# pySTEPS/pysteps

Measured on AMD Instinct MI355X. Metric: Mpixels*leadsteps/s (LK+semilag) at 4096x4096 fp32, higher is better.
Workload: dtype f32

## Files before the change

### pysteps_amd/csrc/lk.hip

```cpp
#include <algorithm>
#include <cmath>
#include <cstring>
#include <functional>
#include <vector>

#include "common.h"

#pragma clang fp contract(off)

namespace psh {
namespace {

enum Stat : int {
  kMinAll = 0,
  kNanCount,
  kMaxAll,
  kMinFeat,
  kMaxFeat,
  kEigMax,
  kNumStats = 8
};

constexpr int kRedBlocks = 1024;

// ... 484 lines not shown
  __syncthreads();
  if (threadIdx.x == 0) {
    for (int w = 1; w < nwaves; ++w) {
      if (what == 0) {
        a = fmin(a, sm[0][w]);
        b += sm[1][w];
      } else {
        a = fmax(a, sm[0][w]);
        b = fmin(b, sm[1][w]);
        c = fmax(c, sm[2][w]);
      }
    }
    if (what == 0) {
      dstats[0] = a;
      stats[kMinAll] = static_cast<float>(a);
      stats[kNanCount] = static_cast<float>(b);
    } else {
      dstats[1] = a;
      dstats[2] = b;
      dstats[3] = c;
      stats[kMaxAll] = static_cast<float>(a);
      stats[kMinFeat] = static_cast<float>(b);
      stats[kMaxFeat] = static_cast<float>(c);
    }
  }
}

__global__ __launch_bounds__(256) void lk_open_bits_f64(const double *__restrict__ img, int m, int n,
                                                        int size_opening, int buffer_mask,
                                                        const float *__restrict__ stats,
                                                        const double *__restrict__ dstats,
                                                        float *__restrict__ clean32, double *__restrict__ clean64,
                                                        double *__restrict__ partial) {
  __shared__ double red[3][4];
  const double mn = dstats[0];
  const int lane = threadIdx.x & 63, wave = threadIdx.x >> 6;
  const int x = blockIdx.x * kOpenColsW - 2 + lane;
  const int yb = blockIdx.y * kOpenRowsWG + wave * kOpenRowsW;
  const bool col_in = x >= 0 && x < n;
  constexpr int kLoad = kOpenRowsW + 4;
  double v[kLoad];
#pragma unroll
  for (int q = 0; q < kLoad; ++q) {
    const int y = yb - 2 + q;
    v[q] = (col_in && y >= 0 && y < m) ? img[static_cast<size_t>(y) * n + x] : 0.0;
  }
  unsigned long long A[kLoad], F[kLoad];
#pragma unroll
  for (int q = 0; q < kLoad; ++q) {
    const int y = yb - 2 + q;
    const bool row_in = y >= 0 && y < m;
    F[q] = __ballot(row_in && col_in && isfinite(v[q]) && v[q] > mn);
    A[q] = F[q] | __ballot(!(row_in && col_in));
  }
  unsigned long long E[kLoad];
#pragma unroll
  for (int q = 1; q < kLoad - 1; ++q) E[q] = F[q] & (A[q] << 1) & (A[q] >> 1) & A[q - 1] & A[q + 1];
  double mx_all = -INFINITY, mn_feat = INFINITY, mx_feat = -INFINITY;
  const int first_row = buffer_mask > 0 ? (stats[kNanCount] > 0.f ? 2 : 1) : 0;
  const bool writer = lane >= 2 && lane < 2 + kOpenColsW && col_in;
#pragma unroll
  for (int q = 2; q < kLoad - 2; ++q) {
    const int y = yb - 2 + q;
    if (y >= m) break;
    const unsigned long long O = E[q] | (E[q] << 1) | (E[q] >> 1) | E[q - 1] | E[q + 1];
    double val = v[q];
    if (size_opening > 0 && ((F[q] >> lane) & 1ull) && !((O >> lane) & 1ull)) val = mn;
    if (writer) {
      if (isfinite(val)) {
        mx_all = fmax(mx_all, val);
        if (y >= first_row) {
          mn_feat = fmin(mn_feat, val);
          mx_feat = fmax(mx_feat, val);
        }
      }
      clean64[static_cast<size_t>(y) * n + x] = val;
      clean32[static_cast<size_t>(y) * n + x] = static_cast<float>(val);
    }
  }
  mx_all = wave_max_d(mx_all);
  mn_feat = wave_min_d(mn_feat);
  mx_feat = wave_max_d(mx_feat);
  if (lane == 0) {
    red[0][wave] = mx_all;
    red[1][wave] = mn_feat;
    red[2][wave] = mx_feat;
  }
  __syncthreads();
  if (threadIdx.x == 0) {
    const int b = blockIdx.y * gridDim.x + blockIdx.x, nb = gridDim.x * gridDim.y;
    partial[b] = fmax(fmax(red[0][0], red[0][1]), fmax(red[0][2], red[0][3]));
    partial[nb + b] = fmin(fmin(red[1][0], red[1][1]), fmin(red[1][2], red[1][3]));
    partial[2 * nb + b] = fmax(fmax(red[2][0], red[2][1]), fmax(red[2][2], red[2][3]));
  }
}

__device__ __forceinline__ unsigned char quantise_f64(double v, double lo, double hi) {
  const double s = (hi - lo) > 1e-8 ? (v - lo) / (hi - lo) * 255.0 : v - lo;
  return static_cast<unsigned char>(static_cast<int>(s));
}

__global__ __launch_bounds__(256) void lk_to_u8_f64(const double *__restrict__ clean, int m, int n, int buffer_mask,
                                                    const float *__restrict__ stats,
                                                    const double *__restrict__ dstats,
                                                    unsigned char *__restrict__ trk, unsigned char *__restrict__ feat) {
  const double fill = dstats[0], hi = dstats[1], flo = dstats[2], fhi = dstats[3];
  const int first_row = buffer_mask > 0 ? (stats[kNanCount] > 0.f ? 2 : 1) : 0;
  const size_t npx = static_cast<size_t>(m) * n;
  const size_t first_feature_px = static_cast<size_t>(first_row) * n;
  const size_t stride = static_cast<size_t>(gridDim.x) * blockDim.x;
  for (size_t p = static_cast<size_t>(blockIdx.x) * blockDim.x + threadIdx.x; p < npx; p += stride) {
    double v = clean[p];
    const bool ok = isfinite(v);
    if (!ok) v = fill;
    trk[p] = quantise_f64(v, fill, hi);
    if (feat) feat[p] = quantise_f64((ok && p >= first_feature_px) ? v : fill, flo, fhi);
  }
}

constexpr int kMaxBlockR = 3;

__device__ __forceinline__ bool px_allowed(const float *__restrict__ clean, int m, int n, int x,
                                           int y, int bm, bool any_nan) {
  if (!any_nan) return true;
  if (bm <= 0) return isfinite(clean[static_cast<size_t>(y) * n + x]);
  const int a = bm / 2;
  for (int j = 0; j < bm; ++j) {
    const int yy = y + j - a;
    if (yy < 0 || yy >= m) continue;
    for (int i = 0; i < bm; ++i) {
      const int xx = x + i - a;
      if (xx < 0 || xx >= n) continue;
      if (!isfinite(clean[static_cast<size_t>(yy) * n + xx])) return false;
    }
  }
  return true;
}

__device__ __forceinline__ float next_lane_f(float v) {
  return __int_as_float(__builtin_amdgcn_update_dpp(0, __float_as_int(v), 0x130 , 0xf, 0xf, true));
}
__device__ __forceinline__ double next_lane_d(double v) {
  const int lo = __builtin_amdgcn_update_dpp(0, __double2loint(v), 0x130, 0xf, 0xf, true);
  const int hi = __builtin_amdgcn_update_dpp(0, __double2hiint(v), 0x130, 0xf, 0xf, true);
  return __hiloint2double(hi, lo);
}
__device__ __forceinline__ bool walk_mirrored(int i, int n) {
  if (i >= 0 && i + 1 < n) return false;
  return reflect101(i + 1, n) != reflect101(reflect101(i, n) + 1, n);
}

constexpr int crn_cols(int block_size) { return 64 - 2 * (block_size / 2 + 1); }

template <int BS, int ROWS>
__global__ __launch_bounds__(256) void lk_corner_response_cols(
    const unsigned char *__restrict__ u8, const float *__restrict__ clean, int m, int n,
    int buffer_mask, const float *__restrict__ stats, float *__restrict__ eig,
    float *__restrict__ partial, Band band, unsigned *__restrict__ slots, int *__restrict__ zero_a, int count_a,
    int *__restrict__ zero_b, int count_b) {
  constexpr int r = BS / 2, H = r + 1, W = crn_cols(BS);
  if (blockIdx.x == 0 && blockIdx.y == 0) {
    for (int i = threadIdx.x; i < count_a; i += 256) zero_a[i] = 0;
    for (int i = threadIdx.x; i < count_b; i += 256) zero_b[i] = 0;
  }
  __shared__ float red[4];
  const int lane = threadIdx.x & 63, wave = __builtin_amdgcn_readfirstlane(threadIdx.x >> 6);
  const int x0 = blockIdx.x * W;
  const int yb = (blockIdx.y * 4 + wave) * ROWS;
  float best = 0.f;
  if (yb < m) {
    const float s = 1.0f / (4.0f * static_cast<float>(BS) * 255.0f), s2 = 2.f * s;
    const int xl = x0 - H + lane;
    const bool neg_x = walk_mirrored(xl + 1, n);
    const float sx = neg_x ? -s : s, sx2 = neg_x ? -s2 : s2;
    const unsigned char *col = u8 + reflect101(xl, n);
    const bool few_rows = m < 2 * H + 2;
    auto row_of = [&](int y) -> int {
      if (few_rows) return reflect101(y, m);
      y = y < 0 ? -y : y;
      return y >= m ? 2 * m - 2 - y : y;
    };
    auto load_row = [&](int i) -> int { return col[static_cast<size_t>(row_of(yb - H + i)) * n]; };
    auto row_terms = [&](int raw, float &hd, float &g) {
      const float a = static_cast<float>(raw);
      const float c = next_lane_f(a);
      const float b = next_lane_f(c);
      hd = b - a;
      g = (a + b) * s + c * s2;
    };
    const bool any_nan = stats[kNanCount] > 0.f;
    const int x = x0 + lane;
    const bool writer = lane < W && x < n;
    const int rows_out = min(ROWS, m - yb);
    const int last_p = rows_out + BS - 1;
    double ring[3][BS], V[3] = {0.0, 0.0, 0.0};
#pragma unroll
    for (int j = 0; j < BS; ++j) ring[0][j] = ring[1][j] = ring[2][j] = 0.0;
    int raw[BS];
    const int raw0 = load_row(0), raw1 = load_row(1);
#pragma unroll
    for (int j = 0; j < BS; ++j) raw[j] = load_row(2 + j);
    float hd_m, hd_0, g_m, g_0;
    row_terms(raw0, hd_m, g_m);
    row_terms(raw1, hd_0, g_0);
    for (int base = 1; base <= last_p; base += BS) {
      int nxt[BS];
#pragma unroll
      for (int j = 0; j < BS; ++j) nxt[j] = load_row(base + BS + 1 + j);
#pragma unroll
      for (int j = 0; j < BS; ++j) {
        const int p = base + j;
        if (p > last_p) break;
        constexpr int kRingBase = 1;
        const int slot = (kRingBase + j) % BS;
        float hd_p, g_p;
        row_terms(raw[j], hd_p, g_p);
        const float dx = (hd_m + hd_p) * sx + hd_0 * sx2;
        float dy = g_p - g_m;
        const int y_seq = yb - H + p;
        const bool row_mirrored = few_rows ? walk_mirrored(y_seq, m) : (y_seq < 0 || y_seq >= m);
        const unsigned row_sign = row_mirrored ? 0x80000000u : 0u;
        dy = __uint_as_float(__float_as_uint(dy) ^ row_sign);
        const double pxx = static_cast<double>(dx * dx), pxy = static_cast<double>(dx * dy);
        const double pyy = static_cast<double>(dy * dy);
        V[0] += pxx - ring[0][slot];
        V[1] += pxy - ring[1][slot];
        V[2] += pyy - ring[2][slot];
        ring[0][slot] = pxx;
        ring[1][slot] = pxy;
        ring[2][slot] = pyy;
        hd_m = hd_0;
        hd_0 = hd_p;
        g_m = g_0;
        g_0 = g_p;
        if (p >= BS) {
          double w0 = V[0], w1 = V[1], w2 = V[2];
          double t0 = V[0], t1 = V[1], t2 = V[2];
#pragma unroll
          for (int c = 0; c < 2 * r; ++c) {
            t0 = next_lane_d(t0);
            t1 = next_lane_d(t1);
            t2 = next_lane_d(t2);
            w0 += t0;
            w1 += t1;
            w2 += t2;
          }
          const int y = yb + p - BS;
          if (writer) {
            const float a = static_cast<float>(w0) * 0.5f, b = static_cast<float>(w1);
            const float c = static_cast<float>(w2) * 0.5f;
            const float e = (a + c) - sqrtf((a - c) * (a - c) + b * b);
            eig[static_cast<size_t>(y) * n + x] = e;
            if (y >= band.lo && y < band.hi && px_allowed(clean, m, n, x, y, buffer_mask, any_nan))
              best = fmaxf(best, fmaxf(e, 0.f));
          }
        }
      }
#pragma unroll
      for (int j = 0; j < BS; ++j) raw[j] = nxt[j];
    }
  }
  best = wave_max(best);
  if (lane == 0) red[wave] = best;
  __syncthreads();
  if (threadIdx.x == 0) {
    const int b = blockIdx.y * gridDim.x + blockIdx.x;
    const float b_max = fmaxf(fmaxf(red[0], red[1]), fmaxf(red[2], red[3]));
    if (slots) {
      slot_max(slots, kSlEig, b, b_max);
    } else {
      partial[b] = b_max;
    }
  }
}

constexpr int kNmsKeys = 64;

using CornerKeyT = unsigned long long;
__device__ __forceinline__ CornerKeyT nms_key(float val, unsigned addr) {
  return (static_cast<CornerKeyT>(__float_as_uint(val)) << 32) | addr;
}
__device__ __forceinline__ float prev_lane_f(float v) {
  return __int_as_float(__builtin_amdgcn_update_dpp(0, __float_as_int(v), 0x138 , 0xf, 0xf, true));
}

template <int BS, int ROWS>
__global__ __launch_bounds__(256) void lk_corner_response_nms(
    const unsigned char *__restrict__ u8, const float *__restrict__ clean, int m, int n, int buffer_mask,
    const float *__restrict__ stats, float quality, CornerKeyT *__restrict__ out, int cap, Band band,
    unsigned *__restrict__ slots, int *__restrict__ zero_b, int count_b) {
  constexpr int r = BS / 2, H = r + 1, W = crn_cols(BS);
  if (blockIdx.x == 0 && blockIdx.y == 0)
    for (int i = threadIdx.x; i < count_b; i += 256) zero_b[i] = 0;
  __shared__ float red[4];
  const int lane = threadIdx.x & 63, wave = __builtin_amdgcn_readfirstlane(threadIdx.x >> 6);
  int *over_count = reinterpret_cast<int *>(slots + kSlCand * kSlots);
  const int fixed_total = static_cast<int>(gridDim.x * gridDim.y) * 4 * kNmsKeys;
  const int my_slots = (static_cast<int>(blockIdx.y * gridDim.x + blockIdx.x) * 4 + wave) * kNmsKeys;
  const int x0 = blockIdx.x * (W - 2) - 1;
  const int yj = (blockIdx.y * 4 + wave) * ROWS;
  const int yb = yj - 1;
  float best = 0.f;
  float known = fmaxf(slots_max(slots, kSlEig), 0.f);
  int held = 0;
  if (yj < m) {
    const float s = 1.0f / (4.0f * static_cast<float>(BS) * 255.0f), s2 = 2.f * s;
    const int xl = x0 - H + lane;
    const bool neg_x = walk_mirrored(xl + 1, n);
    const float sx = neg_x ? -s : s, sx2 = neg_x ? -s2 : s2;
    const unsigned char *col = u8 + reflect101(xl, n);
    const bool few_rows = m < 2 * H + 4;
    auto row_of = [&](int y) -> int {
      if (few_rows) return reflect101(y, m);
      y = y < 0 ? -y : y;
      return y >= m ? 2 * m - 2 - y : y;
    };
    auto load_row = [&](int i) -> int { return col[static_cast<size_t>(row_of(yb - H + i)) * n]; };
    auto row_terms = [&](int raw, float &hd, float &g) {
      const float a = static_cast<float>(raw);
      const float c = next_lane_f(a);
      const float b = next_lane_f(c);
      hd = b - a;
      g = (a + b) * s + c * s2;
    };
    const bool any_nan = stats[kNanCount] > 0.f;
    const int x = x0 + lane;
    const bool in_image_col = lane < W && x >= 0 && x < n;
    const bool judged_col = lane >= 1 && lane < W - 1 && x >= 1 && x < n - 1;
    const int rows_e = min(ROWS + 2, m - yb);
    const int last_p = rows_e + BS - 1;
    double ring[3][BS], V[3] = {0.0, 0.0, 0.0};
#pragma unroll
    for (int j = 0; j < BS; ++j) ring[0][j] = ring[1][j] = ring[2][j] = 0.0;
    int raw[BS];
    const int raw0 = load_row(0), raw1 = load_row(1);
#pragma unroll
    for (int j = 0; j < BS; ++j) raw[j] = load_row(2 + j);
    float hd_m, hd_0, g_m, g_0;
    row_terms(raw0, hd_m, g_m);
    row_terms(raw1, hd_0, g_0);
    float c1 = 0.f, h1 = 0.f, t1 = 0.f, t2 = 0.f;
    for (int base = 1; base <= last_p; base += BS) {
      int nxt[BS];
#pragma unroll
      for (int j = 0; j < BS; ++j) nxt[j] = load_row(base + BS + 1 + j);
#pragma unroll
      for (int j = 0; j < BS; ++j) {
        const int p = base + j;
        if (p > last_p) break;
        constexpr int kRingBase = 1;
        const int slot = (kRingBase + j) % BS;
        float hd_p, g_p;
        row_terms(raw[j], hd_p, g_p);
        const float dx = (hd_m + hd_p) * sx + hd_0 * sx2;
        float dy = g_p - g_m;
        const int y_seq = yb - H + p;
        const bool row_mirrored = few_rows ? walk_mirrored(y_seq, m) : (y_seq < 0 || y_seq >= m);
        const unsigned row_sign = row_mirrored ? 0x80000000u : 0u;
        dy = __uint_as_float(__float_as_uint(dy) ^ row_sign);
        const double pxx = static_cast<double>(dx * dx), pxy = static_cast<double>(dx * dy);
        const double pyy = static_cast<double>(dy * dy);
        V[0] += pxx - ring[0][slot];
        V[1] += pxy - ring[1][slot];
        V[2] += pyy - ring[2][slot];
        ring[0][slot] = pxx;
        ring[1][slot] = pxy;
        ring[2][slot] = pyy;
        hd_m = hd_0;
        hd_0 = hd_p;
        g_m = g_0;
        g_0 = g_p;
        if (p >= BS) {
          double w0 = V[0], w1 = V[1], w2 = V[2];
          double q0 = V[0], q1 = V[1], q2 = V[2];
#pragma unroll
          for (int c = 0; c < 2 * r; ++c) {
            q0 = next_lane_d(q0);
            q1 = next_lane_d(q1);
            q2 = next_lane_d(q2);
            w0 += q0;
            w1 += q1;
            w2 += q2;
          }
          const int y = yb + p - BS;
          const float a = static_cast<float>(w0) * 0.5f, b = static_cast<float>(w1);
          const float c = static_cast<float>(w2) * 0.5f;
          const float e = (a + c) - sqrtf((a - c) * (a - c) + b * b);
          if (in_image_col && y >= 0 && y >= band.lo && y < band.hi && px_allowed(clean, m, n, x, y, buffer_mask, any_nan))
            best = fmaxf(best, fmaxf(e, 0.f));
          if ((p & 7) == 0) known = fmaxf(known, wave_max(best));
          const float h0 = fmaxf(prev_lane_f(e), next_lane_f(e)), t0 = fmaxf(e, h0);
          const int yr = y - 1;
          if (p >= BS + 2 && yr >= yj) {
            bool keep = judged_col && yr >= 1 && yr < m - 1 && yr >= band.lo && yr < band.hi;
            keep = keep && c1 > 0.f && c1 > known * quality;
            keep = keep && !(fmaxf(h1, fmaxf(t2, t0)) > c1);
            keep = keep && px_allowed(clean, m, n, x, yr, buffer_mask, any_nan);
            const unsigned long long mask = __ballot(keep);
            if (mask != 0ull) {
              const int cnt = __popcll(mask);
              int at = held + __popcll(mask & ((1ull << lane) - 1ull));
              if (held + cnt > kNmsKeys) {
                int base = 0;
                const int spill = held + cnt - max(held, kNmsKeys);
                if (lane == 0) base = atomicAdd(over_count, spill);
                base = __shfl(base, 0);
                if (at >= kNmsKeys) at = fixed_total + base + (at - max(held, kNmsKeys)) - my_slots;
              }
              if (keep && my_slots + at < cap) out[my_slots + at] = nms_key(c1, static_cast<unsigned>(yr + band.y_org) * n + x);
              held += cnt;
            }
          }
// ... 560 lines not shown
      for (int r = 0; r < ROWS; ++r) {
        if (r < row_count) {
          const int i00 = from_next_lane(ti[r + 1]), i01 = from_next_lane(i00);
          const int i10 = from_next_lane(ti[r + 2]), i11 = from_next_lane(i10);
          const int g00 = tg[r], g01 = from_next_lane(tg[r]), g10 = tg[r + 1], g11 = from_next_lane(tg[r + 1]);
          if (sample_lane) {
            const int ival = descale(bilin24(i00, i01, i10, i11, w00, w01, w10, w11), 14 - 5);
            const int gx = descale(bilin24(static_cast<short>(g00), static_cast<short>(g01), static_cast<short>(g10),
                                           static_cast<short>(g11), w00, w01, w10, w11), 14);
            const int gy = descale(bilin24(g00 >> 16, g01 >> 16, g10 >> 16, g11 >> 16, w00, w01, w10, w11), 14);
            rI[r] = static_cast<short>(ival);
            rGx[r] = static_cast<short>(gx);
            rGy[r] = static_cast<short>(gy);
            s11 += gx * gx;
            s12 += gx * gy;
            s22 += gy * gy;
          }
        }
      }
    }
    const long long a11 = wave_sum_split_i64(s11), a12 = wave_sum_split_i64(s12), a22 = wave_sum_split_i64(s22);
    if (lane == 0) {
      red[0][wave] = a11;
      red[1][wave] = a12;
      red[2][wave] = a22;
    }
    __syncthreads();
    const float flt_scale = 1.f / 1048576.f;
    const float A11 = static_cast<float>(red[0][0] + red[0][1] + red[0][2] + red[0][3]) * flt_scale;
    const float A12 = static_cast<float>(red[1][0] + red[1][1] + red[1][2] + red[1][3]) * flt_scale;
    const float A22 = static_cast<float>(red[2][0] + red[2][1] + red[2][2] + red[2][3]) * flt_scale;
    float D = A11 * A22 - A12 * A12;
    const float min_eig = (A22 + A11 - sqrtf((A11 - A22) * (A11 - A22) + 4.f * A12 * A12)) /
                          static_cast<float>(2 * win_w * win_h);
    if (min_eig < min_eig_thr || D < 1.1920929e-07f) {
      if (level == 0) ok = false;
      continue;
    }
    D = 1.f / D;
    float qx = nx - half_x, qy = ny - half_y;
    float prev_dx = 0.f, prev_dy = 0.f;
    for (int j = 0; j < max_count; ++j) {
      const int inx = static_cast<int>(floorf(qx)), iny = static_cast<int>(floorf(qy));
      if (iny < L.vlo || iny + win_h + 1 > L.vhi) suspect = true;
      if (inx < -win_w || inx >= L.cols || iny < -win_h || iny >= L.rows) {
        if (level == 0) ok = false;
        break;
      }
      lk_weights(qx - static_cast<float>(inx), qy - static_cast<float>(iny), w00, w01, w10, w11);
      const int y0 = iny + row_first;
      const bool inside = row_count > 0 && inx >= 0 && inx + 63 < L.cols && y0 >= 0 && y0 + ROWS < L.rows &&
                          y0 >= L.row_org && y0 + ROWS - L.row_org < L.rows_stored;
      int tj[ROWS + 1];
      if (inside) {
        const unsigned char *base = L.J + static_cast<size_t>(y0 - L.row_org) * L.cols + (inx + lane);
#pragma unroll
        for (int r = 0; r <= ROWS; ++r) tj[r] = base[static_cast<size_t>(r) * L.cols];
      } else {
        const int xa = reflect101(inx + lane, L.cols);
#pragma unroll
        for (int r = 0; r <= ROWS; ++r)
          tj[r] = L.J[stored_row(L, reflect101(y0 + min(r, max(row_count, 0)), L.rows)) * L.cols + xa];
      }
      int c1 = 0, c2 = 0;
      int right = from_next_lane(tj[0]);
#pragma unroll
      for (int r = 0; r < ROWS; ++r) {
        const int right_below = from_next_lane(tj[r + 1]);
        const int diff = descale(bilin24(tj[r], right, tj[r + 1], right_below, w00, w01, w10, w11), 14 - 5) - rI[r];
        c1 += __mul24(diff, rGx[r]);
        c2 += __mul24(diff, rGy[r]);
        right = right_below;
      }
      const long long b1 = wave_sum_split_i64(c1), b2 = wave_sum_split_i64(c2);
      long long (*rb)[4] = red_b[j & 1];
      if (lane == 0) {
        rb[0][wave] = b1;
        rb[1][wave] = b2;
      }
      __syncthreads();
      const float B1 = static_cast<float>(rb[0][0] + rb[0][1] + rb[0][2] + rb[0][3]) * flt_scale;
      const float B2 = static_cast<float>(rb[1][0] + rb[1][1] + rb[1][2] + rb[1][3]) * flt_scale;
      const float dx = (A12 * B2 - A22 * B1) * D;
      const float dy = (A12 * B1 - A11 * B2) * D;
      qx += dx;
      qy += dy;
      nx = qx + half_x;
      ny = qy + half_y;
      if (dx * dx + dy * dy <= eps2) break;
      if (j > 0 && fabsf(dx + prev_dx) < 0.01f && fabsf(dy + prev_dy) < 0.01f) {
        nx -= dx * 0.5f;
        ny -= dy * 0.5f;
        break;
      }
      prev_dx = dx;
      prev_dy = dy;
    }
    if (level == 0 && ok) {
      const int rx = static_cast<int>(rintf(nx - half_x)), ry = static_cast<int>(rintf(ny - half_y));
      if (ry < L.vlo || ry + win_h + 1 > L.vhi) suspect = true;
      if (rx < -win_w || rx >= L.cols || ry < -win_h || ry >= L.rows) ok = false;
    }
  }
  if (tid == 0) {
    next_pts[p] = make_float2(nx, ny);
    status[p] = (ok ? 1 : 0) | (suspect ? 2 : 0);
  }
}

__global__ __launch_bounds__(256) void lk_pool_append(const float2 *__restrict__ pts,
                                                      const float2 *__restrict__ next_pts,
                                                      const unsigned char *__restrict__ status, int npts,
                                                      const int *__restrict__ npts_dev,
                                                      double2 *__restrict__ pool_xy,
                                                      double2 *__restrict__ pool_uv,
                                                      int *__restrict__ pool_count, int capacity) {
  __shared__ int wave_total[4];
  __shared__ int running;
  const int tid = threadIdx.x, lane = tid & 63, wave = tid >> 6;
  if (npts_dev) npts = min(npts, *npts_dev);
  if (tid == 0) running = *pool_count;
  __syncthreads();
  for (int i0 = 0; i0 < npts; i0 += 256) {
    const int i = i0 + tid;
    const bool keep = i < npts && status[i] != 0;
    const unsigned long long mask = __ballot(keep);
    if (lane == 0) wave_total[wave] = __popcll(mask);
    __syncthreads();
    int pos = running;
    for (int w = 0; w < wave; ++w) pos += wave_total[w];
    pos += __popcll(mask & ((1ull << lane) - 1ull));
    if (keep && pos < capacity) {
      const float2 p = pts[i], q = next_pts[i];
      pool_xy[pos] = make_double2(p.x, p.y);
      pool_uv[pos] = make_double2(static_cast<double>(q.x - p.x), static_cast<double>(q.y - p.y));
    }
    __syncthreads();
    if (tid == 0) running += wave_total[0] + wave_total[1] + wave_total[2] + wave_total[3];
    __syncthreads();
  }
  if (tid == 0) *pool_count = running;
}

}

dim3 lk_open_grid(int m, int n) { return dim3((n + kOpenColsW - 1) / kOpenColsW, (m + kOpenRowsWG32 - 1) / kOpenRowsWG32); }
void launch_lk_open(dim3 grid, hipStream_t stream, const float *img, int m, int n, int size_opening, int buffer_mask,
                    float *stats, float *clean, float *part, Band band, unsigned *slots = nullptr,
                    unsigned long long *keepbits = nullptr) {
  hipLaunchKernelGGL(lk_open_bits, grid, dim3(256), 0, stream, img, m, n, size_opening, buffer_mask, stats, clean, part,
                     band, slots, keepbits);
}

constexpr int kCrnRows = 32;
dim3 lk_response_grid(int m, int n, int block_size) {
  const int w = crn_cols(block_size), rows = 4 * kCrnRows;
  return dim3((n + w - 1) / w, (m + rows - 1) / rows);
}
dim3 lk_response_nms_grid(int m, int n, int block_size) {
  const int w = crn_cols(block_size) - 2, rows = 4 * kCrnRows;
  return dim3((n + w - 1) / w, (m + rows - 1) / rows);
}
int lk_response_nms_fixed_keys(dim3 grid) { return static_cast<int>(grid.x * grid.y) * 4 * kNmsKeys; }
void launch_lk_response_nms(dim3 grid, hipStream_t stream, int block_size, const unsigned char *u8, const float *clean, int m,
                            int n, int buffer_mask, const float *stats, float quality, CornerKeyT *out, int cap, Band band,
                            unsigned *slots, int *zero_b, int count_b) {
#define PSH_NMS_LAUNCH(BS)                                                                                             \
  hipLaunchKernelGGL((lk_corner_response_nms<BS, kCrnRows>), grid, dim3(256), 0, stream, u8, clean, m, n, buffer_mask, \
                     stats, quality, out, cap, band, slots, zero_b, count_b)
  if (block_size == 1) {
    PSH_NMS_LAUNCH(1);
  } else if (block_size == 3) {
    PSH_NMS_LAUNCH(3);
  } else if (block_size == 5) {
    PSH_NMS_LAUNCH(5);
  } else {
    PSH_NMS_LAUNCH(7);
  }
#undef PSH_NMS_LAUNCH
}
void launch_lk_response(dim3 grid, hipStream_t stream, int block_size, const unsigned char *u8, const float *clean, int m,
                        int n, int buffer_mask, const float *stats, float *eig, float *part, Band band,
                        unsigned *slots = nullptr, int *zero_a = nullptr, int count_a = 0, int *zero_b = nullptr,
                        int count_b = 0) {
#define PSH_CRN_LAUNCH(BS)                                                                                          \
  hipLaunchKernelGGL((lk_corner_response_cols<BS, kCrnRows>), grid, dim3(256), 0, stream, u8, clean, m, n, buffer_mask, \
                     stats, eig, part, band, slots, zero_a, count_a, zero_b, count_b)
  if (block_size == 1) {
    PSH_CRN_LAUNCH(1);
  } else if (block_size == 3) {
    PSH_CRN_LAUNCH(3);
  } else if (block_size == 5) {
    PSH_CRN_LAUNCH(5);
  } else {
    PSH_CRN_LAUNCH(7);
  }
#undef PSH_CRN_LAUNCH
}

static int ensure_lk_ws(size_t nbytes, void **ptr) {
  static void *ws = nullptr;
  const int rc = persistent_device(&ws, nbytes);
  *ptr = ws;
  return rc;
}

size_t lk_prepare_ws_bytes(int m, int n, bool f64) {
  const size_t npx = static_cast<size_t>(m) * n;
  if (f64) {
    const dim3 ogrid((n + kOpenColsW - 1) / kOpenColsW, (m + kOpenRowsWG - 1) / kOpenRowsWG);
    return (npx + 2 * static_cast<size_t>(kRedBlocks) + 3 * static_cast<size_t>(ogrid.x * ogrid.y) + 8) * sizeof(double);
  }
  const dim3 ogrid = lk_open_grid(m, n);
  return kSlotBytes + sizeof(float) * (2 * static_cast<size_t>(kRedBlocks) + 3 * static_cast<size_t>(ogrid.x * ogrid.y));
}
size_t lk_slot_bytes() { return kSlotBytes; }
size_t lk_keepbits_bytes(int m, int n) { return static_cast<size_t>(m) * lk_open_grid(m, n).x * sizeof(unsigned long long); }

int lk_prepare_on(hipStream_t stream, void *ws, const void *frame_dev, bool f64, int m, int n, int size_opening,
                  int buffer_mask, float *clean_dev, unsigned char *track_u8_dev, unsigned char *feature_u8_dev,
                  float *stats_dev, unsigned *slots_cleared, unsigned long long *keepbits) {
  if (m <= 0 || n <= 0) return fail(PSH_EINVAL, "lk_prepare: invalid shape (%d,%d)", m, n);
  if (!frame_dev || !track_u8_dev || !stats_dev || !ws) return fail(PSH_EINVAL, "lk_prepare: NULL pointer");
  if (!clean_dev && (f64 || !keepbits)) return fail(PSH_EINVAL, "lk_prepare: NULL pointer");
  if (size_opening != 0 && size_opening != 3)
    return fail(PSH_EUNSUPPORTED, "lk_prepare: size_opening %d not implemented (0 or 3)", size_opening);
  const size_t npx = static_cast<size_t>(m) * n;
  if (!f64) {
    const float *frame = static_cast<const float *>(frame_dev);
    const dim3 ogrid = lk_open_grid(m, n);
    unsigned *own_slots = static_cast<unsigned *>(ws);
    float *part1 = reinterpret_cast<float *>(static_cast<char *>(ws) + kSlotBytes);
    float *part2 = part1 + 2 * kRedBlocks;
    unsigned *slots = slots_cleared;
    if (!slots) {
      slots = own_slots;
      const hipError_t e = hipMemsetAsync(slots, 0, kSlotBytes, stream);
      if (e != hipSuccess) return fail(PSH_EHIP, "lk_prepare: clearing the statistic slots failed: %s", hipGetErrorString(e));
    }
    hipLaunchKernelGGL(lk_stats1, dim3(kRedBlocks), dim3(256), 0, stream, frame, npx, part1, slots);
    if (clean_dev) {
      launch_lk_open(ogrid, stream, frame, m, n, size_opening, buffer_mask, stats_dev, clean_dev, part2, Band{0, 0, m}, slots);
      const int qgrid = static_cast<int>(std::min<size_t>((npx / 4 + 255) / 256 + 1, 4096));
      hipLaunchKernelGGL(lk_to_u8, dim3(qgrid), dim3(256), 0, stream, clean_dev, m, n, buffer_mask, stats_dev, track_u8_dev,
                         feature_u8_dev, 0, static_cast<const unsigned *>(slots));
    } else {
      launch_lk_open(ogrid, stream, frame, m, n, size_opening, buffer_mask, stats_dev, nullptr, part2, Band{0, 0, m}, slots,
                     keepbits);
      const dim3 qgrid((n + 1023) / 1024, (m + kU8Rows - 1) / kU8Rows);
      const bool vec = n % 4 == 0 && reinterpret_cast<uintptr_t>(frame) % 16 == 0 &&
                       reinterpret_cast<uintptr_t>(track_u8_dev) % 4 == 0 && reinterpret_cast<uintptr_t>(feature_u8_dev) % 4 == 0;
      if (vec) {
        hipLaunchKernelGGL(lk_to_u8_bits<true>, qgrid, dim3(256), 0, stream, frame, keepbits, static_cast<int>(ogrid.x), m, n,
                           buffer_mask, stats_dev, track_u8_dev, feature_u8_dev, static_cast<const unsigned *>(slots));
      } else {
        hipLaunchKernelGGL(lk_to_u8_bits<false>, qgrid, dim3(256), 0, stream, frame, keepbits, static_cast<int>(ogrid.x), m, n,
                           buffer_mask, stats_dev, track_u8_dev, feature_u8_dev, static_cast<const unsigned *>(slots));
      }
    }
  } else {
    const double *frame = static_cast<const double *>(frame_dev);
    const dim3 ogrid((n + kOpenColsW - 1) / kOpenColsW, (m + kOpenRowsWG - 1) / kOpenRowsWG);
    const int nb_open = ogrid.x * ogrid.y;
    double *clean64 = static_cast<double *>(ws);
    double *part1 = clean64 + npx, *part2 = part1 + 2 * kRedBlocks, *dstats = part2 + 3 * nb_open;
    hipLaunchKernelGGL(lk_stats1_f64, dim3(kRedBlocks), dim3(256), 0, stream, frame, npx, part1);
    hipLaunchKernelGGL(lk_final_f64, dim3(1), dim3(kFinalThreads), 0, stream, part1, kRedBlocks, 0, stats_dev, dstats);
    hipLaunchKernelGGL(lk_open_bits_f64, ogrid, dim3(256), 0, stream, frame, m, n, size_opening, buffer_mask, stats_dev,
                       dstats, clean_dev, clean64, part2);
    hipLaunchKernelGGL(lk_final_f64, dim3(1), dim3(kFinalThreads), 0, stream, part2, nb_open, 1, stats_dev, dstats);
    const int qgrid = static_cast<int>(std::min<size_t>((npx + 255) / 256, 8192));
    hipLaunchKernelGGL(lk_to_u8_f64, dim3(qgrid), dim3(256), 0, stream, clean64, m, n, buffer_mask, stats_dev, dstats,
                       track_u8_dev, feature_u8_dev);
  }
  const hipError_t e = hipGetLastError();
  if (e != hipSuccess) return fail(PSH_EHIP, "lk_prepare launch failed: %s", hipGetErrorString(e));
  return PSH_OK;
}


}

using psh::ctx;
using psh::fail;

extern "C" {

int psh_lk_prepare_dev(const float *frame_dev, int m, int n, int size_opening, int buffer_mask,
                       float *clean_dev, unsigned char *track_u8_dev,
                       unsigned char *feature_u8_dev, float *stats_dev) {
  PSH_REQUIRE_INIT();
  psh::Context &c = ctx();
  std::lock_guard<std::recursive_mutex> lock(c.mu);
  PSH_HIP(hipSetDevice(c.device));
  if (m <= 0 || n <= 0) return fail(PSH_EINVAL, "lk_prepare: invalid shape (%d,%d)", m, n);
  void *ws = nullptr;
  if (int rc = psh::ensure_lk_ws(psh::lk_prepare_ws_bytes(m, n, false), &ws)) return rc;
  return psh::lk_prepare_on(c.stream, ws, frame_dev, false, m, n, size_opening, buffer_mask, clean_dev, track_u8_dev,
                            feature_u8_dev, stats_dev);
}

int psh_lk_prepare_f64_dev(const double *frame_dev, int m, int n, int size_opening, int buffer_mask,
                           float *clean_dev, unsigned char *track_u8_dev,
                           unsigned char *feature_u8_dev, float *stats_dev) {
  PSH_REQUIRE_INIT();
  psh::Context &c = ctx();
  std::lock_guard<std::recursive_mutex> lock(c.mu);
  PSH_HIP(hipSetDevice(c.device));
  if (m <= 0 || n <= 0) return fail(PSH_EINVAL, "lk_prepare: invalid shape (%d,%d)", m, n);
  void *blk = nullptr;
  if (int rc = psh_malloc(&blk, psh::lk_prepare_ws_bytes(m, n, true))) return rc;
  const int rc = psh::lk_prepare_on(c.stream, blk, frame_dev, true, m, n, size_opening, buffer_mask, clean_dev,
                                    track_u8_dev, feature_u8_dev, stats_dev);
  (void)psh_free(blk);
  return rc;
}

static int check_band(const char *who, int m, int n, int e0, int e1, int r0, int r1) {
  if (m <= 0 || n <= 0 || e0 < 0 || e1 > m || e0 >= e1 || r0 < e0 || r1 > e1 || r0 > r1)
    return fail(PSH_EINVAL, "%s: rows [%d,%d) / band [%d,%d) do not fit a %d-row frame", who, r0, r1, e0, e1, m);
  return PSH_OK;
}

int psh_lk_band_stats_dev(const float *frame_dev, int m, int n, int r0, int r1, float *stats_dev) {
  PSH_REQUIRE_INIT();
  if (!frame_dev || !stats_dev) return fail(PSH_EINVAL, "lk_band_stats: NULL pointer");
  if (int rc = check_band("lk_band_stats", m, n, r0, r1, r0, r1)) return rc;
  psh::Context &c = ctx();
  std::lock_guard<std::recursive_mutex> lock(c.mu);
  PSH_HIP(hipSetDevice(c.device));
  void *ws = nullptr;
  if (int rc = psh::ensure_lk_ws(sizeof(float) * 2 * psh::kRedBlocks, &ws)) return rc;
  float *part = static_cast<float *>(ws);
  hipLaunchKernelGGL(psh::lk_stats1, dim3(psh::kRedBlocks), dim3(256), 0, c.stream,
                     frame_dev + static_cast<size_t>(r0) * n, static_cast<size_t>(r1 - r0) * n, part,
                     static_cast<unsigned *>(nullptr));
  hipLaunchKernelGGL(psh::lk_stats1_final, dim3(1), dim3(psh::kFinalThreads), 0, c.stream, part, psh::kRedBlocks, stats_dev);
  PSH_HIP(hipGetLastError());
  return PSH_OK;
// ... 796 lines not shown
```

Baseline: 282,100.

## Process two columns per lane in corner response kernel with packed loads

Restructures the corner-response kernel so each lane handles C=2 adjacent columns, with packed 16-bit byte loads on interior tiles and vectorized float2 stores. The horizontal box sum becomes a sliding window across lane-shifted values. The ring buffer now stores fp32 products instead of doubles to cut register pressure, and rows per wave go from 32 to 36. The goals are fewer DPP shuffles and memory transactions per pixel and less halo waste, at the cost of more registers per lane and more complex boundary handling.

```diff
diff --git a/pysteps_amd/csrc/lk.hip b/pysteps_amd/csrc/lk.hip
--- a/pysteps_amd/csrc/lk.hip
+++ b/pysteps_amd/csrc/lk.hip
@@ -660,112 +660,208 @@
 
 constexpr int crn_cols(int block_size) { return 64 - 2 * (block_size / 2 + 1); }
 
-template <int BS, int ROWS>
+constexpr int crn_geom_e(int r, int c) { return ((c - 1 - r) % c + c) % c; }
+template <int BS, int C>
+struct CrnGeom {
+  static constexpr int r = BS / 2;
+  static constexpr int E = crn_geom_e(r, C);
+  static constexpr int lead = 1 + E + r;
+  static constexpr int NT = C + 2 * r;
+  static constexpr int px_lanes = (E + C + 1) / C;
+  static constexpr int look = (NT - 1) / C + px_lanes;
+  static constexpr int lanes = 64 - look;
+  static constexpr int cols = C * lanes;
+  static_assert(lead % C == 0, "loads and stores of a lane are aligned together");
+};
+constexpr int kCrnC = 2;
+constexpr int kCrnRows = 36;
+constexpr int crn_strip_cols(int block_size) {
+  const int r = block_size / 2, e = crn_geom_e(r, kCrnC);
+  return kCrnC * (64 - ((kCrnC + 2 * r - 1) / kCrnC + (e + kCrnC + 1) / kCrnC));
+}
+
+__device__ __forceinline__ unsigned next_lane_u(unsigned v) {
+  return static_cast<unsigned>(__builtin_amdgcn_update_dpp(0, static_cast<int>(v), 0x130 , 0xf, 0xf, true));
+}
+
+template <int BS, int C, int ROWS, bool PACKED>
+__device__ __forceinline__ float crn_walk(const unsigned char *__restrict__ u8, const float *__restrict__ clean, int m,
+                                          int n, int buffer_mask, bool any_nan, float *__restrict__ eig, Band band,
+                                          int x0, int yb, int lane) {
+  using G = CrnGeom<BS, C>;
+  constexpr int r = G::r, H = r + 1, E = G::E, NT = G::NT;
+  const float s = 1.0f / (4.0f * static_cast<float>(BS) * 255.0f), s2 = 2.f * s;
+  const int q = x0 - G::lead + C * lane;
+  int off[C];
+  float sx[C], sx2[C];
+#pragma unroll
+  for (int j = 0; j < C; ++j) {
+    off[j] = PACKED ? q + j : reflect101(q + j, n);
+    const bool neg_x = !PACKED && walk_mirrored(q + 1 + E + j, n);
+    sx[j] = neg_x ? -s : s;
+    sx2[j] = neg_x ? -s2 : s2;
+  }
+  const bool few_rows = m < 2 * H + 2;
+  auto row_of = [&](int y) -> int {
+    if (few_rows) return reflect101(y, m);
+    y = y < 0 ? -y : y;
+    y = y >= m ? 2 * m - 2 - y : y;
+    return min(max(y, 0), m - 1);
+  };
+  auto load_row = [&](int i) -> unsigned {
+    const unsigned char *row = u8 + static_cast<size_t>(row_of(yb - H + i)) * n;
+    if (PACKED) {
+      if (C == 4) return *reinterpret_cast<const unsigned *>(row + q);
+      return *reinterpret_cast<const unsigned short *>(row + q);
+    }
+    unsigned w = 0;
+#pragma unroll
+    for (int k = 0; k < C; ++k) w |= static_cast<unsigned>(row[off[k]]) << (8 * k);
+    return w;
+  };
+  auto row_terms = [&](unsigned raw, float (&hd)[C], float (&g)[C]) {
+    unsigned w[G::px_lanes + 1];
+    w[0] = raw;
+#pragma unroll
+    for (int i = 1; i <= G::px_lanes; ++i) w[i] = next_lane_u(w[i - 1]);
+    float px[C + 2];
+#pragma unroll
+    for (int k = 0; k < C + 2; ++k) px[k] = static_cast<float>((w[(E + k) / C] >> (8 * ((E + k) % C))) & 0xffu);
+#pragma unroll
+    for (int j = 0; j < C; ++j) {
+      hd[j] = px[j + 2] - px[j];
+      g[j] = (px[j] + px[j + 2]) * s + px[j + 1] * s2;
+    }
+  };
+  const int x = x0 + C * lane;
+  const bool writer = lane < G::lanes && x < n;
+  const bool store_vec = (n % C) == 0 && (reinterpret_cast<uintptr_t>(eig) & (4 * C - 1)) == 0;
+  const int rows_out = min(ROWS, m - yb);
+  const int last_p = rows_out + BS - 1;
+  float best = 0.f;
+  float ring[3][BS][C];
+  double V[3][C];
+#pragma unroll
+  for (int j = 0; j < C; ++j) {
+    V[0][j] = V[1][j] = V[2][j] = 0.0;
+#pragma unroll
+    for (int k = 0; k < BS; ++k) ring[0][k][j] = ring[1][k][j] = ring[2][k][j] = 0.f;
+  }
+  unsigned raw[BS];
+  const unsigned raw0 = load_row(0), raw1 = load_row(1);
+#pragma unroll
+  for (int j = 0; j < BS; ++j) raw[j] = load_row(2 + j);
+  float hd_m[C], hd_0[C], g_m[C], g_0[C];
+  row_terms(raw0, hd_m, g_m);
+  row_terms(raw1, hd_0, g_0);
+  for (int base = 1; base <= last_p; base += BS) {
+    unsigned nxt[BS];
+#pragma unroll
+    for (int j = 0; j < BS; ++j) nxt[j] = load_row(base + BS + 1 + j);
+#pragma unroll
+    for (int jr = 0; jr < BS; ++jr) {
+      const int p = base + jr;
+      if (p > last_p) break;
+      constexpr int kRingBase = 1;
+      const int slot = (kRingBase + jr) % BS;
+      float hd_p[C], g_p[C];
+      row_terms(raw[jr], hd_p, g_p);
+      const int y_seq = yb - H + p;
+      const bool row_mirrored = few_rows ? walk_mirrored(y_seq, m) : (y_seq < 0 || y_seq >= m);
+      const unsigned row_sign = row_mirrored ? 0x80000000u : 0u;
+#pragma unroll
+      for (int j = 0; j < C; ++j) {
+        const float dx = (hd_m[j] + hd_p[j]) * sx[j] + hd_0[j] * sx2[j];
+        float dy = g_p[j] - g_m[j];
+        dy = __uint_as_float(__float_as_uint(dy) ^ row_sign);
+        const float pxx = dx * dx, pxy = dx * dy, pyy = dy * dy;
+        V[0][j] += static_cast<double>(pxx) - static_cast<double>(ring[0][slot][j]);
+        V[1][j] += static_cast<double>(pxy) - static_cast<double>(ring[1][slot][j]);
+        V[2][j] += static_cast<double>(pyy) - static_cast<double>(ring[2][slot][j]);
+        ring[0][slot][j] = pxx;
+        ring[1][slot][j] = pxy;
+        ring[2][slot][j] = pyy;
+        hd_m[j] = hd_0[j];
+        hd_0[j] = hd_p[j];
+        g_m[j] = g_0[j];
+        g_0[j] = g_p[j];
+      }
+      if (p >= BS) {
+        float w[3][C];
+#pragma unroll
+        for (int k = 0; k < 3; ++k) {
+          double t[NT];
+#pragma unroll
+          for (int i = 0; i < NT; ++i) t[i] = i < C ? V[k][i] : next_lane_d(t[i - C]);
+          double acc = t[0];
+#pragma unroll
+          for (int i = 1; i <= 2 * r; ++i) acc += t[i];
+          w[k][0] = static_cast<float>(acc);
+#pragma unroll
+          for (int j = 1; j < C; ++j) {
+            acc += t[j + 2 * r];
+            acc -= t[j - 1];
+            w[k][j] = static_cast<float>(acc);
+          }
+        }
+        float e[C];
+#pragma unroll
+        for (int j = 0; j < C; ++j) {
+          const float a = w[0][j] * 0.5f, b = w[1][j], c = w[2][j] * 0.5f;
+          e[j] = (a + c) - sqrtf((a - c) * (a - c) + b * b);
+        }
+        const int y = yb + p - BS;
+        if (writer) {
+          float *out = eig + static_cast<size_t>(y) * n + x;
+          if (store_vec) {
+            if (C == 4) {
+              *reinterpret_cast<float4 *>(out) = make_float4(e[0], e[1], e[2], e[3]);
+            } else {
+              *reinterpret_cast<float2 *>(out) = make_float2(e[0], e[1]);
+            }
+          } else {
+#pragma unroll
+            for (int j = 0; j < C; ++j)
+              if (x + j < n) out[j] = e[j];
+          }
+          if (y >= band.lo && y < band.hi) {
+#pragma unroll
+            for (int j = 0; j < C; ++j)
+              if (x + j < n && px_allowed(clean, m, n, x + j, y, buffer_mask, any_nan)) best = fmaxf(best, fmaxf(e[j], 0.f));
+          }
+        }
+      }
+    }
+#pragma unroll
+    for (int j = 0; j < BS; ++j) raw[j] = nxt[j];
+  }
+  return best;
+}
+
+template <int BS, int C, int ROWS>
 __global__ __launch_bounds__(256) void lk_corner_response_cols(
     const unsigned char *__restrict__ u8, const float *__restrict__ clean, int m, int n,
     int buffer_mask, const float *__restrict__ stats, float *__restrict__ eig,
     float *__restrict__ partial, Band band, unsigned *__restrict__ slots, int *__restrict__ zero_a, int count_a,
     int *__restrict__ zero_b, int count_b) {
-  constexpr int r = BS / 2, H = r + 1, W = crn_cols(BS);
+  using G = CrnGeom<BS, C>;
   if (blockIdx.x == 0 && blockIdx.y == 0) {
     for (int i = threadIdx.x; i < count_a; i += 256) zero_a[i] = 0;
     for (int i = threadIdx.x; i < count_b; i += 256) zero_b[i] = 0;
   }
   __shared__ float red[4];
   const int lane = threadIdx.x & 63, wave = __builtin_amdgcn_readfirstlane(threadIdx.x >> 6);
-  const int x0 = blockIdx.x * W;
+  const int x0 = blockIdx.x * G::cols;
   const int yb = (blockIdx.y * 4 + wave) * ROWS;
   float best = 0.f;
   if (yb < m) {
-    const float s = 1.0f / (4.0f * static_cast<float>(BS) * 255.0f), s2 = 2.f * s;
-    const int xl = x0 - H + lane;
-    const bool neg_x = walk_mirrored(xl + 1, n);
-    const float sx = neg_x ? -s : s, sx2 = neg_x ? -s2 : s2;
-    const unsigned char *col = u8 + reflect101(xl, n);
-    const bool few_rows = m < 2 * H + 2;
-    auto row_of = [&](int y) -> int {
-      if (few_rows) return reflect101(y, m);
-      y = y < 0 ? -y : y;
-      return y >= m ? 2 * m - 2 - y : y;
-    };
-    auto load_row = [&](int i) -> int { return col[static_cast<size_t>(row_of(yb - H + i)) * n]; };
-    auto row_terms = [&](int raw, float &hd, float &g) {
-      const float a = static_cast<float>(raw);
-      const float c = next_lane_f(a);
-      const float b = next_lane_f(c);
-      hd = b - a;
-      g = (a + b) * s + c * s2;
-    };
     const bool any_nan = stats[kNanCount] > 0.f;
-    const int x = x0 + lane;
-    const bool writer = lane < W && x < n;
-    const int rows_out = min(ROWS, m - yb);
-    const int last_p = rows_out + BS - 1;
-    double ring[3][BS], V[3] = {0.0, 0.0, 0.0};
-#pragma unroll
-    for (int j = 0; j < BS; ++j) ring[0][j] = ring[1][j] = ring[2][j] = 0.0;
-    int raw[BS];
-    const int raw0 = load_row(0), raw1 = load_row(1);
-#pragma unroll
-    for (int j = 0; j < BS; ++j) raw[j] = load_row(2 + j);
-    float hd_m, hd_0, g_m, g_0;
-    row_terms(raw0, hd_m, g_m);
-    row_terms(raw1, hd_0, g_0);
-    for (int base = 1; base <= last_p; base += BS) {
-      int nxt[BS];
-#pragma unroll
-      for (int j = 0; j < BS; ++j) nxt[j] = load_row(base + BS + 1 + j);
-#pragma unroll
-      for (int j = 0; j < BS; ++j) {
-        const int p = base + j;
-        if (p > last_p) break;
-        constexpr int kRingBase = 1;
-        const int slot = (kRingBase + j) % BS;
-        float hd_p, g_p;
-        row_terms(raw[j], hd_p, g_p);
-        const float dx = (hd_m + hd_p) * sx + hd_0 * sx2;
-        float dy = g_p - g_m;
-        const int y_seq = yb - H + p;
-        const bool row_mirrored = few_rows ? walk_mirrored(y_seq, m) : (y_seq < 0 || y_seq >= m);
-        const unsigned row_sign = row_mirrored ? 0x80000000u : 0u;
-        dy = __uint_as_float(__float_as_uint(dy) ^ row_sign);
-        const double pxx = static_cast<double>(dx * dx), pxy = static_cast<double>(dx * dy);
-        const double pyy = static_cast<double>(dy * dy);
-        V[0] += pxx - ring[0][slot];
-        V[1] += pxy - ring[1][slot];
-        V[2] += pyy - ring[2][slot];
-        ring[0][slot] = pxx;
-        ring[1][slot] = pxy;
-        ring[2][slot] = pyy;
-        hd_m = hd_0;
-        hd_0 = hd_p;
-        g_m = g_0;
-        g_0 = g_p;
-        if (p >= BS) {
-          double w0 = V[0], w1 = V[1], w2 = V[2];
-          double t0 = V[0], t1 = V[1], t2 = V[2];
-#pragma unroll
-          for (int c = 0; c < 2 * r; ++c) {
-            t0 = next_lane_d(t0);
-            t1 = next_lane_d(t1);
-            t2 = next_lane_d(t2);
-            w0 += t0;
-            w1 += t1;
-            w2 += t2;
-          }
-          const int y = yb + p - BS;
-          if (writer) {
-            const float a = static_cast<float>(w0) * 0.5f, b = static_cast<float>(w1);
-            const float c = static_cast<float>(w2) * 0.5f;
-            const float e = (a + c) - sqrtf((a - c) * (a - c) + b * b);
-            eig[static_cast<size_t>(y) * n + x] = e;
-            if (y >= band.lo && y < band.hi && px_allowed(clean, m, n, x, y, buffer_mask, any_nan))
-              best = fmaxf(best, fmaxf(e, 0.f));
-          }
-        }
-      }
-#pragma unroll
-      for (int j = 0; j < BS; ++j) raw[j] = nxt[j];
+    const int first = x0 - G::lead;
+    const bool packed = (n & 3) == 0 && (reinterpret_cast<uintptr_t>(u8) & 3) == 0 && first >= 0 && first + 64 * C <= n;
+    if (packed) {
+      best = crn_walk<BS, C, ROWS, true>(u8, clean, m, n, buffer_mask, any_nan, eig, band, x0, yb, lane);
+    } else {
+      best = crn_walk<BS, C, ROWS, false>(u8, clean, m, n, buffer_mask, any_nan, eig, band, x0, yb, lane);
     }
   }
   best = wave_max(best);
@@ -1632,13 +1728,13 @@
                      band, slots, keepbits);
 }
 
-constexpr int kCrnRows = 32;
+constexpr int kNmsRows = 32;
 dim3 lk_response_grid(int m, int n, int block_size) {
-  const int w = crn_cols(block_size), rows = 4 * kCrnRows;
+  const int w = crn_strip_cols(block_size), rows = 4 * kCrnRows;
   return dim3((n + w - 1) / w, (m + rows - 1) / rows);
 }
 dim3 lk_response_nms_grid(int m, int n, int block_size) {
-  const int w = crn_cols(block_size) - 2, rows = 4 * kCrnRows;
+  const int w = crn_cols(block_size) - 2, rows = 4 * kNmsRows;
   return dim3((n + w - 1) / w, (m + rows - 1) / rows);
 }
 int lk_response_nms_fixed_keys(dim3 grid) { return static_cast<int>(grid.x * grid.y) * 4 * kNmsKeys; }
@@ -1646,7 +1742,7 @@
                             int n, int buffer_mask, const float *stats, float quality, CornerKeyT *out, int cap, Band band,
                             unsigned *slots, int *zero_b, int count_b) {
 #define PSH_NMS_LAUNCH(BS)                                                                                             \
-  hipLaunchKernelGGL((lk_corner_response_nms<BS, kCrnRows>), grid, dim3(256), 0, stream, u8, clean, m, n, buffer_mask, \
+  hipLaunchKernelGGL((lk_corner_response_nms<BS, kNmsRows>), grid, dim3(256), 0, stream, u8, clean, m, n, buffer_mask, \
                      stats, quality, out, cap, band, slots, zero_b, count_b)
   if (block_size == 1) {
     PSH_NMS_LAUNCH(1);
@@ -1664,7 +1760,7 @@
                         unsigned *slots = nullptr, int *zero_a = nullptr, int count_a = 0, int *zero_b = nullptr,
                         int count_b = 0) {
 #define PSH_CRN_LAUNCH(BS)                                                                                          \
-  hipLaunchKernelGGL((lk_corner_response_cols<BS, kCrnRows>), grid, dim3(256), 0, stream, u8, clean, m, n, buffer_mask, \
+  hipLaunchKernelGGL((lk_corner_response_cols<BS, kCrnC, kCrnRows>), grid, dim3(256), 0, stream, u8, clean, m, n, buffer_mask, \
                      stats, eig, part, band, slots, zero_a, count_a, zero_b, count_b)
   if (block_size == 1) {
     PSH_CRN_LAUNCH(1);
```

Result: no change. 284,300 (median of 6 runs) (+0.8%).
